# nimblephysics/nimblephysics

Hardware: AMD Instinct MI355X
Metric: worlds*timesteps/sec fwd+bwd (higher is better)
Workload: dtype f64; 1 GPU; Atlas 20-DOF (free root + 14 revolutes, arms welded) standing on the ground box, 8 frictional foot-corner contacts (24 LCP rows), pose q[0]=-pi/2 q[4]=-0.01 + N(0,0.02^2) joint noise; batch=4096 worlds/GPU; fwd+bwd through the C ABI, cold LCP start each step; ONE model handle in deferred-join mode (its slices run on the handle's own streams, the per-slice loss on them); n_dofs=20, contacts=8, lcp_rows=24, worlds_per_gpu=4096, saved_record_bytes_per_world_step=26720, rccl_world_size=0, devices_visible=1, device_of_rank0=0, gpu_max_hw_queues=4, collective=1 all-gather of the shared-control gradient per timed region

## Files before the change

nimblephysics_amd/csrc/coop_dantzig_dev.hpp:

```cpp
#pragma once
#include "coop_dev.hpp"

namespace NBL_NS {

template <int I> struct IntTag { static constexpr int value = I; };

DEV void coopPin24(double (&a)[MAXR]) {
#if defined(__HIP_DEVICE_COMPILE__)
  static_assert(MAXR % 8 == 0, "groups of eight");
#pragma unroll
  for (int g = 0; g < MAXR; g += 8)
    asm volatile("" : "+v"(a[g]), "+v"(a[g + 1]), "+v"(a[g + 2]), "+v"(a[g + 3]), "+v"(a[g + 4]), "+v"(a[g + 5]), "+v"(a[g + 6]), "+v"(a[g + 7]));
#endif
}

#if defined(NBL_CASCADE_TIMING) && defined(__HIPCC__)
__device__ unsigned long long g_dzStat[16];
__device__ unsigned long long g_dzStatSlow[16];
#ifndef NBL_DZ_SLOW
#define NBL_DZ_SLOW 300000
#endif
#endif
#if defined(NBL_CASCADE_TIMING) && defined(__HIP_DEVICE_COMPILE__)
#define DZ_T0() long long dzT = clock64(); long long dzAcc[12] = {0, 0, 0, 0, 0, 0, 0, 0, 0, 0, 0, 0}
#define DZ_ADD(k) do { const long long dzN = clock64(); dzAcc[k] += dzN - dzT; dzT = dzN; } while (0)
#define DZ_CNT(k) do { dzAcc[k] += 1; } while (0)
#define DZ_FLUSH() do { if (ln == 0) { long long dzTot = 0; for (int dzK = 0; dzK < 8; dzK++) dzTot += dzAcc[dzK];                      \
                                        for (int dzK = 0; dzK < 12; dzK++) atomicAdd(&g_dzStat[dzK], (unsigned long long)dzAcc[dzK]);           \
                                        if (dzTot > NBL_DZ_SLOW) for (int dzK = 0; dzK < 12; dzK++) atomicAdd(&g_dzStatSlow[dzK], (unsigned long long)dzAcc[dzK]); } } while (0)
#else
#define DZ_T0() do { } while (0)
#define DZ_ADD(k) do { } while (0)
#define DZ_CNT(k) do { } while (0)
#define DZ_FLUSH() do { } while (0)
#endif

struct PgsLds {
  double A[MAXR * CLD];
  double v[4][MAXR];
};

struct CascadeLds {
  double A[MAXR * CLD];
  double L[MAXR * CLD];
  double v[4][MAXR];
  double d[MAXR];
  int iv[2][MAXR];
};

struct CoopLcpRow {
  double x, b, lo, hi;
  int findex;
};

#if defined(__HIP_DEVICE_COMPILE__)
constexpr unsigned dzLanes(int from, int to) { return from >= to ? 0u : (unsigned)(((1ull << to) - 1ull) & ~((1ull << from) - 1ull)); }
template <unsigned SW>
DEV void dzSwitchStep(double& acc, double rhs, unsigned long long all) {
  asm volatile("s_mov_b64 exec, %[sw]\n\t"
               "v_add_f64 %[acc], %[rhs], -%[acc]\n\t"
               "s_mov_b64 exec, %[all]"
               : [acc] "+v"(acc)
               : [rhs] "v"(rhs), [sw] "n"(SW), [all] "s"(all));
}
template <unsigned YM, unsigned ZM>
DEV void dzSubstStep(double& acc, double l, double xk, unsigned long long all) {
  double t;
  if constexpr (YM != 0u && ZM != 0u) {
    asm volatile("v_mul_f64 %[t], %[l], %[xk]\n\t"
                 "s_mov_b64 exec, %[ym]\n\t"
                 "v_add_f64 %[acc], %[acc], -%[t]\n\t"
                 "s_mov_b64 exec, %[zm]\n\t"
                 "v_add_f64 %[acc], %[acc], %[t]\n\t"
                 "s_mov_b64 exec, %[all]"
                 : [acc] "+v"(acc), [t] "=&v"(t)
                 : [l] "v"(l), [xk] "s"(xk), [ym] "n"(YM), [zm] "n"(ZM), [all] "s"(all));
  } else if constexpr (YM != 0u) {
    asm volatile("v_mul_f64 %[t], %[l], %[xk]\n\t"
                 "s_mov_b64 exec, %[ym]\n\t"
                 "v_add_f64 %[acc], %[acc], -%[t]\n\t"
                 "s_mov_b64 exec, %[all]"
                 : [acc] "+v"(acc), [t] "=&v"(t)
                 : [l] "v"(l), [xk] "s"(xk), [ym] "n"(YM), [all] "s"(all));
  } else if constexpr (ZM != 0u) {
    asm volatile("v_mul_f64 %[t], %[l], %[xk]\n\t"
                 "s_mov_b64 exec, %[zm]\n\t"
                 "v_add_f64 %[acc], %[acc], %[t]\n\t"
                 "s_mov_b64 exec, %[all]"
                 : [acc] "+v"(acc), [t] "=&v"(t)
                 : [l] "v"(l), [xk] "s"(xk), [zm] "n"(ZM), [all] "s"(all));
  }
}
template <int K, class W>
DEV void dzL1BlockStep(const W& w, double& acc, double rhs, const double (&lrow)[MAXR], unsigned long long all) {
  if constexpr (K % 4 == 0) dzSwitchStep<dzLanes(K, K + 4)>(acc, rhs, all);
  const double xk = w.bcast(acc, K);
  dzSubstStep<dzLanes(K + 1, (K | 3) + 1), dzLanes((K | 3) + 1, 32)>(acc, lrow[K], xk, all);
}
template <int K, class W>
DEV void dzL1TailStep(const W& w, double& acc, double rhs, const double (&lrow)[MAXR], unsigned long long all) {
  dzSwitchStep<dzLanes(K, K + 1)>(acc, rhs, all);
  const double xk = w.bcast(acc, K);
  dzSubstStep<0u, dzLanes(K + 1, 32)>(acc, lrow[K], xk, all);
}
template <int J, class W>
DEV void dzL1Blocks(const W& w, double& acc, double rhs, const double (&lrow)[MAXR], int nC, int nb4, unsigned long long all) {
  if constexpr (4 * J < MAXR) {
    if (4 * J < nb4) {
      dzL1BlockStep<4 * J>(w, acc, rhs, lrow, all);
      dzL1BlockStep<4 * J + 1>(w, acc, rhs, lrow, all);
      dzL1BlockStep<4 * J + 2>(w, acc, rhs, lrow, all);
      dzL1BlockStep<4 * J + 3>(w, acc, rhs, lrow, all);
      dzL1Blocks<J + 1>(w, acc, rhs, lrow, nC, nb4, all);
    } else if (4 * J < nC) {
      dzL1TailStep<4 * J>(w, acc, rhs, lrow, all);
      if (4 * J + 1 < nC) {
        dzL1TailStep<4 * J + 1>(w, acc, rhs, lrow, all);
        if (4 * J + 2 < nC) dzL1TailStep<4 * J + 2>(w, acc, rhs, lrow, all);
      }
    }
  }
}
template <int RHO, int K, class W>
DEV void dzL1TBlockStep(const W& w, double& acc, double rhs, const double (&lcol)[MAXR], unsigned long long all) {
  constexpr int B0 = RHO + 4 * ((K - RHO) / 4);
  if constexpr (K == B0 + 3) dzSwitchStep<dzLanes(B0, B0 + 4)>(acc, rhs, all);
  const double xk = w.bcast(acc, K);
  dzSubstStep<dzLanes(B0, K), dzLanes(0, B0)>(acc, lcol[K], xk, all);
}
template <int K, class W>
DEV void dzL1TTailStep(const W& w, double& acc, double rhs, const double (&lcol)[MAXR], unsigned long long all) {
  dzSwitchStep<dzLanes(K, K + 1)>(acc, rhs, all);
  const double xk = w.bcast(acc, K);
  dzSubstStep<0u, dzLanes(0, K)>(acc, lcol[K], xk, all);
}
template <int RHO, int J, class W>
DEV void dzL1TBlocks(const W& w, double& acc, double rhs, const double (&lcol)[MAXR], int nC, unsigned long long all) {
  if constexpr (J >= 0) {
    if constexpr (RHO + 4 * J + 3 < MAXR) {
      if (RHO + 4 * J + 3 < nC) {
        dzL1TBlockStep<RHO, RHO + 4 * J + 3>(w, acc, rhs, lcol, all);
        dzL1TBlockStep<RHO, RHO + 4 * J + 2>(w, acc, rhs, lcol, all);
        dzL1TBlockStep<RHO, RHO + 4 * J + 1>(w, acc, rhs, lcol, all);
        dzL1TBlockStep<RHO, RHO + 4 * J>(w, acc, rhs, lcol, all);
      }
    }
    dzL1TBlocks<RHO, J - 1>(w, acc, rhs, lcol, nC, all);
  } else {
    if constexpr (RHO >= 3) dzL1TTailStep<2>(w, acc, rhs, lcol, all);
    if constexpr (RHO >= 2) dzL1TTailStep<1>(w, acc, rhs, lcol, all);
    if constexpr (RHO >= 1) dzL1TTailStep<0>(w, acc, rhs, lcol, all);
  }
}
#endif

template <class W>
DEV int coopDantzig(const W& w, CascadeLds& C, int n, CoopLcpRow& row) {
#if defined(__clang__)
#pragma clang fp contract(off)
#endif
  const int ln = w.lane();
  const bool on = ln < n;
  const int me = on ? ln : 0;
  DZ_T0();
  DZ_CNT(8);
  double x = 0.0, ww = 0.0, b = on ? row.b : 0.0, lo = on ? row.lo : 0.0, hi = on ? row.hi : 0.0, dx = 0.0, dw = 0.0;
  int st = 0, fidx = on ? row.findex : -1, p = me;
  int Cv = 0;
  double ell = 0.0, Dell = 0.0;
  int nC = 0, nN = 0;
  auto swapProblem = [&](int i1, int i2) {
    if (i1 == i2) return;
    if (on) { const double t = C.A[i1 * CLD + ln]; C.A[i1 * CLD + ln] = C.A[i2 * CLD + ln]; C.A[i2 * CLD + ln] = t; }
    w.sync();
    if (on) { const double t = C.A[ln * CLD + i1]; C.A[ln * CLD + i1] = C.A[ln * CLD + i2]; C.A[ln * CLD + i2] = t; }
    w.sync();
    const int src = ln == i1 ? i2 : (ln == i2 ? i1 : ln);
    x = w.shfl(x, src); b = w.shfl(b, src); ww = w.shfl(ww, src); lo = w.shfl(lo, src); hi = w.shfl(hi, src);
    p = w.shflI(p, src); st = w.shflI(st, src); fidx = w.shflI(fidx, src);
  };
  {
    const uint64_t fricBits = w.ballot(on && fidx >= 0);
    int atEnd = 0;
    for (int k = n - 1; k >= 0; k--) {
      if ((fricBits >> k) & 1ull) {
        const int i2 = n - 1 - atEnd;
        if (k != i2) {
          const int pk = w.bcastI(p, k), pi = w.bcastI(p, i2), fk = w.bcastI(fidx, k), f2 = w.bcastI(fidx, i2);
          const bool isK = ln == k, isI2 = ln == i2;
          p = isK ? pi : (isI2 ? pk : p);
          fidx = isK ? f2 : (isI2 ? fk : fidx);
        }
        atEnd++;
      }
    }
    double col[MAXR];
#pragma unroll
    for (int r = 0; r < MAXR; r++) {
      const int pr = w.bcastI(p, r < n ? r : 0);
      const int hiI = pr >= p ? pr : p, loI = pr >= p ? p : pr;
      const double av = C.A[hiI * CLD + loI];
      col[r] = (on && r < n) ? av : 0.0;
    }
    w.sync();
    if (ln < MAXR) {
#pragma unroll
      for (int r = 0; r < MAXR; r++) C.A[r * CLD + ln] = col[r];
    }
    b = w.shfl(b, p); lo = w.shfl(lo, p); hi = w.shfl(hi, p);
    w.sync();
  }
  auto seqRange = [&](double prod, int from, int to) -> double {
    double s = 0.0;
    int k = from;
#pragma unroll 1
    for (; k + 4 <= to; k += 4) {
      const double t0 = w.bcast(prod, k), t1 = w.bcast(prod, k + 1), t2 = w.bcast(prod, k + 2), t3 = w.bcast(prod, k + 3);
      s = s + t0; s = s + t1; s = s + t2; s = s + t3;
    }
#pragma unroll 1
    for (; k < to; k++) s = s + w.bcast(prod, k);
    return s;
  };
#ifdef NBL_SEQSUM_LDS
  auto seqSum2 = [&](double prod, int mid, int to, double& s1, double& s2) {
    w.sync();
    if (ln < MAXR) { C.v[2][ln] = ln < mid ? prod : 0.0; C.v[3][ln] = (ln >= mid && ln < to) ? prod : 0.0; }
    w.sync();
    s1 = 0.0; s2 = 0.0;
#pragma unroll
    for (int k4 = 0; k4 < MAXR; k4 += 4) {
      if (k4 < to) {
#pragma unroll
        for (int k = k4; k < k4 + 4; k++) { s1 = s1 + C.v[2][k]; s2 = s2 + C.v[3][k]; }
      }
    }
  };
#else
  auto seqSum2 = [&](double prod, int mid, int to, double& s1, double& s2) {
    s1 = seqRange(prod, 0, mid);
    s2 = seqRange(prod, mid, to);
  };
#endif
#ifdef NBL_SEQSUM_LDS
  auto seqSum = [&](double prod, int from, int to) -> double { double s1, s2; seqSum2(prod, to, to, s1, s2); return s1; };
#else
  auto seqSum = [&](double prod, int from, int to) -> double { return seqRange(prod, from, to); };
#endif
  auto solveL1 = [&](double rhs) -> double {
    const bool act = ln < nC;
    const int nb4 = nC & ~3;
    const int i0 = (ln < nb4) ? (ln & ~3) : ln;
    double lrow[MAXR];
#pragma unroll
    for (int k = 0; k < MAXR; k++) lrow[k] = C.L[me * CLD + k];
    coopPin24(lrow);
#if defined(__HIP_DEVICE_COMPILE__)
    if constexpr (MAXR <= 32) {
      double acc = 0.0;
      const unsigned long long all = __builtin_amdgcn_read_exec();
      dzL1Blocks<0>(w, acc, rhs, lrow, nC, nb4, all);
      return ln < nC ? acc : rhs;
    }
#endif
    double Z = 0.0, y = rhs;
#pragma unroll
    for (int k = 0; k < MAXR; k++) {
      if (k < nC) {
        if (k == i0) y = rhs - Z;
        const double xk = w.bcast(y, k);
        const double t = lrow[k] * xk;
        if (act && k < i0) Z = Z + t;
        if (k >= i0 && k < ln) y = y - t;
      }
    }
    return y;
  };
  auto solveL1T = [&](double rhs) -> double {
    const bool act = ln < nC;
    const int jr = nC - 1 - ln;
    const int nb4 = nC & ~3;
    const int i0 = (jr < nb4) ? (jr & ~3) : jr;
    double lcol[MAXR];
#pragma unroll
    for (int k = 0; k < MAXR; k++) lcol[k] = C.L[k * CLD + me];
    coopPin24(lcol);
#if defined(__HIP_DEVICE_COMPILE__)
    if constexpr (MAXR <= 32) {
      double acc = 0.0;
      const unsigned long long all = __builtin_amdgcn_read_exec();
      const int rho = nC & 3;
      constexpr int JTOP = MAXR / 4 - 1;
      if (rho == 0) dzL1TBlocks<0, JTOP>(w, acc, rhs, lcol, nC, all);
      else if (rho == 1) dzL1TBlocks<1, JTOP>(w, acc, rhs, lcol, nC, all);
      else if (rho == 2) dzL1TBlocks<2, JTOP>(w, acc, rhs, lcol, nC, all);
      else dzL1TBlocks<3, JTOP>(w, acc, rhs, lcol, nC, all);
      return ln < nC ? acc : rhs;
    }
#endif
    double Z = 0.0, y = rhs;
#pragma unroll
    for (int k = MAXR - 1; k >= 0; k--) {
      if (k < nC) {
        const int kr = nC - 1 - k;
        if (kr == i0) y = rhs - Z;
        const double xk = w.bcast(y, k);
        const double t = lcol[k] * xk;
        if (act && kr < i0) Z = Z + t;
        if (act && kr >= i0 && kr < jr) y = y - t;
      }
    }
    return y;
  };
  auto solveEll = [&](int i) {
    const double rhs = ln < nC ? C.A[i * CLD + Cv] : 0.0;
    Dell = solveL1(rhs);
    ell = ln < nC ? Dell * C.d[me] : 0.0;
  };
  auto solve1 = [&](int i, int dir) {
    if (nC == 0) return;
    solveEll(i);
    const double t = solveL1T(ell);
    w.sync();
    if (ln < nC) C.v[1][Cv] = dir > 0 ? -t : t;
    w.sync();
    dx = ln < nC ? C.v[1][me] : dx;
  };
  auto appendFactorRow = [&](int i) {
    const double aii = C.A[i * CLD + i];
    if (nC > 0) {
      if (ln < nC) C.L[nC * CLD + ln] = ell;
      const double dot = seqSum(ell * Dell, 0, nC);
      if (ln == 0) C.d[nC] = 1.0 / (aii - dot);
    } else if (ln == 0) C.d[0] = 1.0 / aii;
    w.sync();
  };
  auto ldltAddTL = [&](int r, int n2, double a) {
    const int nn = n2 - r;
    if (nn < 2) return;
    const bool act = ln >= r && ln < n2;
    const int pl = ln - r;
    const double SQ = 0.70710678118654752440;
    double W1 = (act && pl >= 1) ? a * SQ : 0.0, W2 = W1;
    const double a0 = w.bcast(a, r);
    const double W11 = (0.5 * a0 + 1.0) * SQ, W21 = (0.5 * a0 - 1.0) * SQ;
    double alpha1 = 1.0, alpha2 = 1.0;
    {
      double dee = C.d[r];
      double alphanew = alpha1 + (W11 * W11) * dee;
      dee /= alphanew;
      const double gamma1 = W11 * dee;
      dee *= alpha1;
      alpha1 = alphanew;
      alphanew = alpha2 - (W21 * W21) * dee;
      dee /= alphanew;
      alpha2 = alphanew;
      const double k1 = 1.0 - W21 * gamma1;
      const double k2 = W21 * gamma1 * W11 - W21;
      if (act && pl >= 1) {
        const double Wp = W1, el = C.L[me * CLD + r];
        W1 = Wp - W11 * el;
        W2 = k1 * Wp + k2 * el;
      }
    }
#pragma unroll 1
    for (int j = 1; j < nn; j++) {
      const double k1 = w.bcast(W1, r + j), k2 = w.bcast(W2, r + j);
      double dee = C.d[r + j];
      double alphanew = alpha1 + (k1 * k1) * dee;
      dee /= alphanew;
      const double gamma1 = k1 * dee;
      dee *= alpha1;
      alpha1 = alphanew;
      alphanew = alpha2 - (k2 * k2) * dee;
      dee /= alphanew;
      const double gamma2 = k2 * dee;
      dee *= alpha2;
      w.sync();
      if (ln == 0) C.d[r + j] = dee;
      alpha2 = alphanew;
      if (act && pl > j) {
        double el = C.L[me * CLD + r + j];
        double Wp = W1 - k1 * el;
        el += gamma1 * Wp;
        W1 = Wp;
        Wp = W2 - k2 * el;
        el -= gamma2 * Wp;
        W2 = Wp;
        C.L[me * CLD + r + j] = el;
      }
    }
    w.sync();
  };
  auto ldltRemove = [&](int n2, int r) {
    if (r == n2 - 1) return;
    const bool act = ln >= r && ln < n2;
    const int Cr = w.bcastI(Cv, r);
    const double ga = C.A[(act ? Cv : 0) * CLD + Cr];
    double a;
    if (r == 0) a = -ga;
    else {
      if (ln < r) C.v[2][ln] = C.L[r * CLD + ln] / C.d[ln];
      w.sync();
      double s = 0.0;
#pragma unroll 1
      for (int k = 0; k < r; k++) s = s + C.L[me * CLD + k] * C.v[2][k];
      a = s - ga;
    }
    if (ln == r) a += 1.0;
    ldltAddTL(r, n2, act ? a : 0.0);
    double lrow[MAXR];
    const int src = ln >= r ? ln + 1 : ln;
    const int srcc = src < MAXR ? src : MAXR - 1;
#pragma unroll
    for (int k = 0; k < MAXR; k++) lrow[k] = C.L[srcc * CLD + (k >= r ? (k + 1 < MAXR ? k + 1 : MAXR - 1) : k)];
    const double dsrc = C.d[srcc];
    w.sync();
    if (ln < n2 - 1) {
#pragma unroll
      for (int k = 0; k < MAXR; k++) C.L[ln * CLD + k] = lrow[k];
      C.d[ln] = dsrc;
    }
    w.sync();
  };
  auto removeFromC = [&](int i) {
    const int j = __builtin_ctzll(w.ballot(ln < nC && Cv == i));
    ldltRemove(nC, j);
    const int k = __builtin_ctzll(w.ballot(ln < nC && Cv == nC - 1));
    if (ln == k) Cv = i;
    const int cNext = w.shflI(Cv, ln + 1);
    if (ln >= j) Cv = cNext;
    swapProblem(i, nC - 1);
    nN++; nC--;
  };
  bool hitFirstFriction = false;
#ifdef NBL_DZ_COUNTS
  int dzIters = 0, dzRemovals = 0, dzTransfers = 0;
#endif
  DZ_ADD(0);
  for (int i = 0; i < n; ++i) {
    DZ_CNT(9);
    const int fi = w.bcastI(fidx, i);
    if (!hitFirstFriction && fi >= 0) {
      if (on) C.v[0][p] = x;
      w.sync();
      if (on && ln >= i) {
        const double wfk = C.v[0][fidx >= 0 ? fidx : 0];
        if (wfk == 0) { hi = 0; lo = 0; }
        else { hi = fabs(hi * wfk); lo = -hi; }
      }
      w.sync();
      hitFirstFriction = true;
    }
    {
      const double pr = on ? C.A[i * CLD + me] * x : 0.0;
      double sC, sN;
      seqSum2(pr, nC, nC + nN, sC, sN);
      const double s = sC + sN - w.bcast(b, i);
      if (ln == i) ww = s;
    }
    DZ_ADD(1);
    const double wi0 = w.bcast(ww, i), loi = w.bcast(lo, i), hii = w.bcast(hi, i);
    if (loi == 0 && wi0 >= 0) { if (ln == i) st = 0; nN++; }
    else if (hii == 0 && wi0 <= 0) { if (ln == i) st = 1; nN++; }
    else if (wi0 == 0) {
      if (nC > 0) solveEll(i);
      appendFactorRow(i); swapProblem(nC, i); if (ln == nC) Cv = nC; nC++;
    } else {
      for (;;) {
        const double wi = w.bcast(ww, i);
        const int dir = (wi <= 0) ? 1 : -1;
        const double dirf = dir;
        DZ_CNT(10);
#ifdef NBL_DZ_COUNTS
        dzIters++;
#endif
        solve1(i, dir);
        DZ_ADD(2);
        {
          double arow[MAXR];
#pragma unroll
          for (int j = 0; j < MAXR; j++) arow[j] = C.A[me * CLD + j];
          const double ai = C.A[me * CLD + i];
          coopPin24(arow);
          const double dxz = ln < nC ? dx : 0.0;
          double s = 0.0;
#pragma unroll
          for (int j4 = 0; j4 < MAXR; j4 += 4) {
            if (j4 < nC) {
              const double x0 = w.bcast(dxz, j4), x1 = w.bcast(dxz, j4 + 1), x2 = w.bcast(dxz, j4 + 2), x3 = w.bcast(dxz, j4 + 3);
              const double p0 = arow[j4] * x0, p1 = arow[j4 + 1] * x1, p2 = arow[j4 + 2] * x2, p3 = arow[j4 + 3] * x3;
              s = s + p0; s = s + p1; s = s + p2; s = s + p3;
            }
          }
          const bool inN = ln >= nC && ln < nC + nN;
          if (inN) dw = dir > 0 ? s + ai : s - ai;
          if (ln == i) dw = s + ai * dirf;
        }
        DZ_ADD(3);
        const bool inN = ln >= nC && ln < nC + nN, inC = ln < nC, isI = ln == i;
        const bool dn = dx < 0;
        const double num = (isI || inN) ? -ww : ((dn ? lo : hi) - x);
        const double den = (isI || inN) ? dw : dx;
        const double q = num / den;
        double s = INFINITY;
        int cmd = 0;
        if (isI) {
          s = q; cmd = 1;
          if (dir > 0) { if (hi < INFINITY) { const double s2 = (hi - x) * dirf; if (s2 < s) { s = s2; cmd = 3; } } }
          else { if (lo > -INFINITY) { const double s2 = (lo - x) * dirf; if (s2 < s) { s = s2; cmd = 2; } } }
        } else if (inN) {
          if (((st == 0) ? dw < 0 : dw > 0) && !(lo == 0 && hi == 0)) { s = q; cmd = 4; }
        } else if (inC) {
          if (dn && lo > -INFINITY) { s = q; cmd = 5; }
          if (dx > 0 && hi < INFINITY) { s = q; cmd = 6; }
        }
        const double sOwn = w.bcast(s, i);
        if (sOwn != sOwn) { row.x = 0.0; DZ_FLUSH(); return -1; }
        const double sMin = w.template minRows<MAXR>(cmd != 0 ? s : INFINITY);
        const uint64_t tie = w.ballot(cmd != 0 && s == sMin);
        if (tie == 0ull) { row.x = 0.0; DZ_FLUSH(); return -1; }
        int best;
        {
          const uint64_t mi = tie & (1ull << i);
          const uint64_t maskN = nN > 0 ? (((1ull << nN) - 1ull) << nC) : 0ull;
          const uint64_t maskC = nC > 0 ? ((1ull << nC) - 1ull) : 0ull;
          if (mi) best = i;
          else if (tie & maskN) best = __builtin_ctzll(tie & maskN);
          else best = __builtin_ctzll((tie & maskC) ? (tie & maskC) : tie);
        }
        const int cmdB = w.bcastI(cmd, best);
        if (sMin <= 0.0) { row.x = 0.0; DZ_FLUSH(); return 0; }
        const int si = best;
        DZ_ADD(4);
        if (ln < nC) x = x + sMin * dx;
        if (ln == i) x = x + sMin * dirf;
        if (ln >= nC && ln < nC + nN) ww = ww + sMin * dw;
        if (ln == i) ww = ww + sMin * dw;
        switch (cmdB) {
          case 1: if (ln == i) ww = 0; appendFactorRow(i); swapProblem(nC, i); if (ln == nC) Cv = nC; nC++; break;
          case 2: if (ln == i) { x = lo; st = 0; } nN++; break;
          case 3: if (ln == i) { x = hi; st = 1; } nN++; break;
          case 4:
            if (ln == si) ww = 0;
            if (nC > 0) solveEll(si);
            appendFactorRow(si); swapProblem(nC, si); if (ln == nC) Cv = nC; nN--; nC++; break;
          case 5: if (ln == si) { x = lo; st = 0; } removeFromC(si); break;
          case 6: if (ln == si) { x = hi; st = 1; } removeFromC(si); break;
        }
        if (cmdB >= 5) DZ_CNT(11);
#ifdef NBL_DZ_COUNTS
        if (cmdB >= 5) dzRemovals++;
        if (cmdB == 4) dzTransfers++;
#endif
        if (cmdB >= 5) DZ_ADD(7);
        else DZ_ADD(5);
        if (cmdB <= 3) break;
      }
    }
    DZ_ADD(6);
  }
  w.sync();
  if (on) C.v[0][p] = x;
  w.sync();
  row.x = on ? C.v[0][ln] : 0.0;
  w.sync();
  DZ_FLUSH();
#ifdef NBL_DZ_COUNTS
  row.x = ln == 0 ? (double)dzIters : (ln == 1 ? (double)dzRemovals : (ln == 2 ? (double)dzTransfers : 0.0));
#endif
  return 1;
}

template <class W, class LDS>
DEV void coopRemoveRow(const W& w, LDS& C, int n, int col, CoopLcpRow& row) {
  const int ln = w.lane();
  if (ln < n) for (int j = col; j + 1 < n; j++) C.A[ln * CLD + j] = C.A[ln * CLD + j + 1];
  w.sync();
  if (ln < n) for (int i = col; i + 1 < n; i++) C.A[i * CLD + ln] = C.A[(i + 1) * CLD + ln];
  w.sync();
  const double x1 = w.shfl(row.x, ln + 1), b1 = w.shfl(row.b, ln + 1), l1 = w.shfl(row.lo, ln + 1), h1 = w.shfl(row.hi, ln + 1);
  const int f1 = w.shflI(row.findex, ln + 1);
  if (ln >= col && ln + 1 < n) { row.x = x1; row.b = b1; row.lo = l1; row.hi = h1; row.findex = f1; }
}

template <class W, class LDS>
DEV int coopKeepRows(const W& w, LDS& C, int n, uint64_t keep, CoopLcpRow& row, int& mapTo) {
  const int ln = w.lane();
  const int nNew = __builtin_popcountll(keep);
  auto newIdx = [&](int p) -> int { return __builtin_popcountll(keep & ((1ull << p) - 1ull)); };
  const bool kept = ln < n && ((keep >> ln) & 1ull);
  w.sync();
  if (kept) C.v[0][newIdx(ln)] = (double)ln;
  w.sync();
  const int src = ln < nNew ? (int)C.v[0][ln] : 0;
  double col[MAXR];
  {
    uint64_t mm = keep;
#pragma unroll
    for (int j = 0; j < MAXR; j++) {
      if (j < nNew) {
        const int sj = __builtin_ctzll(mm);
        mm &= mm - 1ull;
        col[j] = C.A[src * CLD + sj];
      }
    }
  }
  w.sync();
  if (kept) { const int t = newIdx(ln); C.v[0][t] = row.x; C.v[1][t] = row.b; C.v[2][t] = row.lo; C.v[3][t] = row.hi; }
  const int fOld = w.shflI(row.findex, src);
  if (ln < nNew) {
#pragma unroll
    for (int j = 0; j < MAXR; j++) if (j < nNew) C.A[ln * CLD + j] = col[j];
  }
  w.sync();
  if (ln < nNew) {
    row.x = C.v[0][ln]; row.b = C.v[1][ln]; row.lo = C.v[2][ln]; row.hi = C.v[3][ln];
    row.findex = fOld >= 0 ? newIdx(fOld) : -1;
  }
  if (mapTo >= 0) mapTo = ((keep >> mapTo) & 1ull) ? newIdx(mapTo) : -1;
  w.sync();
  return nNew;
}

template <class W, class LDS>
DEV int coopLcpReduce(const W& w, LDS& C, int n, CoopLcpRow& row, int& mapTo) {
  const double TH = 1e-4;
  const int ln = w.lane();
  for (;;) {
    int ma = -1, mb = -1;
    for (int a = 0; a < n - 1; a++) {
      const double ba = w.bcast(row.b, a), ha = w.bcast(row.hi, a), la = w.bcast(row.lo, a);
      const int fa = w.bcastI(row.findex, a);
      const bool cand = ln > a && ln < n && fabs(ba - row.b) < TH && fa == row.findex && ha == row.hi && la == row.lo;
      if (w.ballot(cand) == 0ull) continue;
      double d2 = 0;
      const int bcol = ln < n ? ln : 0;
#pragma unroll
      for (int r = 0; r < MAXR; r++) {
        const double dr = C.A[r * CLD + a] - C.A[r * CLD + bcol];
        const double d = (r < n) ? dr : 0.0;
        d2 += d * d;
      }
      const uint64_t mm = w.ballot(cand && d2 < TH);
      if (mm) { ma = a; mb = __builtin_ctzll(mm); break; }
    }
    if (ma < 0) break;
    if (ln < n) C.A[ln * CLD + ma] *= 2.0;
    if (row.findex == mb) row.findex = ma;
    else if (row.findex > mb) row.findex -= 1;
    w.sync();
    coopRemoveRow(w, C, n, mb, row);
    n -= 1;
    if (mapTo == mb) mapTo = ma;
    else if (mapTo > mb) mapTo -= 1;
  }
  return n;
}

template <class W, class LDS>
DEV int coopLcpRemoveFriction(const W& w, LDS& C, int n, CoopLcpRow& row, int& mapTo) {
  const int ln = w.lane();
  return coopKeepRows(w, C, n, w.ballot(ln < n && row.findex == -1), row, mapTo);
}

#if defined(__HIP_DEVICE_COMPILE__)
#define NBL_PGS_OWN_NOFRIC                        \
        "s_mov_b64 exec, %[lane]\n\t"             \
        "v_add_f64 %[t0], %[x], %[r]\n\t"         \
        "v_max_f64 %[t0], %[t0], %[cL]\n\t"       \
        "v_min_f64 %[t0], %[t0], %[cH]\n\t"       \
        "v_add_f64 %[d], %[t0], -%[x]\n\t"        \
        "v_mov_b64 %[x], %[t0]\n\t"               \
        "s_mov_b64 exec, %[all]"
#define NBL_PGS_OWN_FRIC                          \
        "s_mov_b64 exec, %[lane]\n\t"             \
        "v_add_f64 %[t0], %[x], %[r]\n\t"         \
        "v_mul_f64 %[t1], %[cL], %[xf]\n\t"       \
        "v_max_f64 %[t0], %[t0], %[t1]\n\t"       \
        "v_mul_f64 %[t1], %[cH], %[xf]\n\t"       \
        "v_min_f64 %[t0], %[t0], %[t1]\n\t"       \
        "v_add_f64 %[d], %[t0], -%[x]\n\t"        \
        "v_mov_b64 %[x], %[t0]\n\t"               \
        "s_mov_b64 exec, %[all]"
template <int I, bool NOFRIC>
DEV void pgsOwnRow(double& x, double r, double xf, double cL, double cH, double& d, unsigned long long all) {
  double t0, t1;
  if constexpr (I < 32) {
    if constexpr (NOFRIC)
      asm volatile(NBL_PGS_OWN_NOFRIC : [x] "+v"(x), [d] "+v"(d), [t0] "=&v"(t0)
                   : [r] "v"(r), [cL] "v"(cL), [cH] "v"(cH), [lane] "n"(1u << (I & 31)), [all] "s"(all));
    else
      asm volatile(NBL_PGS_OWN_FRIC : [x] "+v"(x), [d] "+v"(d), [t0] "=&v"(t0), [t1] "=&v"(t1)
                   : [r] "v"(r), [xf] "v"(xf), [cL] "v"(cL), [cH] "v"(cH), [lane] "n"(1u << (I & 31)), [all] "s"(all));
  } else {
    const unsigned long long laneMask = 1ull << I;
    if constexpr (NOFRIC)
      asm volatile(NBL_PGS_OWN_NOFRIC : [x] "+v"(x), [d] "+v"(d), [t0] "=&v"(t0)
                   : [r] "v"(r), [cL] "v"(cL), [cH] "v"(cH), [lane] "s"(laneMask), [all] "s"(all));
    else
      asm volatile(NBL_PGS_OWN_FRIC : [x] "+v"(x), [d] "+v"(d), [t0] "=&v"(t0), [t1] "=&v"(t1)
                   : [r] "v"(r), [xf] "v"(xf), [cL] "v"(cL), [cH] "v"(cH), [lane] "s"(laneMask), [all] "s"(all));
  }
}
template <int I>
DEV void pgsFollowRow(double& xf, double& r, int fi, double ds, double narowI, unsigned long long all) {
  asm volatile("v_cmpx_eq_u32_e32 vcc, %[row], %[fi]\n\t"
               "s_nop 0\n\t"
               "v_add_f64 %[xf], %[xf], %[ds]\n\t"
               "s_mov_b64 exec, %[all]\n\t"
               "v_fmac_f64_e32 %[r], %[ds], %[na]"
               : [xf] "+v"(xf), [r] "+v"(r)
               : [fi] "v"(fi), [ds] "s"(ds), [na] "v"(narowI), [row] "n"(I), [all] "s"(all)
               : "vcc");
}
template <bool FIRST>
DEV bool pgsSweepBad(double x, double d, double thrFirst, double relTol, double epsDiv) {
  unsigned long long bad;
  if constexpr (FIRST) {
    asm volatile("v_cmp_gt_f64_e64 %[bad], |%[d]|, %[thr]" : [bad] "=s"(bad) : [d] "v"(d), [thr] "v"(thrFirst));
  } else {
    double t2;
    unsigned long long sc;
    asm volatile("v_mul_f64 %[t2], |%[x]|, %[rel]\n\t"
                 "v_cmp_gt_f64_e64 %[sc], |%[x]|, %[eps]\n\t"
                 "v_cmp_gt_f64_e64 %[bad], |%[d]|, %[t2]\n\t"
                 "s_and_b64 %[bad], %[bad], %[sc]"
                 : [bad] "=&s"(bad), [sc] "=&s"(sc), [t2] "=&v"(t2)
                 : [x] "v"(x), [d] "v"(d), [rel] "v"(relTol), [eps] "v"(epsDiv)
                 : "scc");
  }
  return bad != 0ull;
}
#else
template <int I, bool NOFRIC>
DEV void pgsOwnRow(double& x, double r, double xf, double cL, double cH, double& d, unsigned long long) {
  const double xi = NOFRIC ? fmin(fmax(x + r, cL), cH) : fmin(fmax(x + r, cL * xf), cH * xf);
  d = xi - x;
  x = xi;
}
template <int I>
DEV void pgsFollowRow(double& xf, double& r, int fi, double ds, double narowI, unsigned long long) {
  if (fi == I) xf += ds;
  r = fma(narowI, ds, r);
}
template <bool FIRST>
DEV bool pgsSweepBad(double x, double d, double thrFirst, double relTol, double epsDiv) {
  return FIRST ? fabs(d) > thrFirst : (fabs(x) > epsDiv && fabs(d) > relTol * fabs(x));
}
#endif

template <int I0, int I1, class F, class T>
DEV void pgsRowRange(F& rowStep, T tag) {
  if constexpr (I0 < I1) {
    rowStep(IntTag<I0>{}, tag);
    pgsRowRange<I0 + 1, I1>(rowStep, tag);
  }
}

template <bool NOFRIC = false, class W, class LDS>
DEV bool coopPgs(const W& w, LDS& C, int n, CoopLcpRow& row) {
  const int maxIteration = 30;
  const double dxTh = 1e-6, relTol = 1e-3, epsDiv = 1e-9;
  const int ln = w.lane();
  const bool on = ln < n;
  const int me = on ? ln : 0;
  double narow[MAXR];
#pragma unroll
  for (int j = 0; j < MAXR; j++) { const double av = C.A[me * CLD + j]; narow[j] = (on && j < n) ? av : 0.0; }
  const double aii = on ? C.A[me * CLD + me] : 1.0;
  const bool inOrder = on && !(aii < epsDiv);
  const double sc = inOrder ? 1.0 / aii : 1.0;
  const double nsc = -sc;
#pragma unroll
  for (int j = 0; j < MAXR; j++) narow[j] *= nsc;
  double x = on ? row.x : 0.0;
  double r0 = row.b * sc, r1 = 0.0;
#pragma unroll
  for (int j = 0; j < MAXR; j += 2) {
    r0 = fma(narow[j], j < n ? w.bcast(x, j) : 0.0, r0);
    r1 = fma(narow[j + 1], j + 1 < n ? w.bcast(x, j + 1) : 0.0, r1);
  }
  double r = r0 + r1;
  const int fi = on ? row.findex : -1;
  const bool fric = fi >= 0;
  const double cH = !inOrder ? 0.0 : row.hi, cL = !inOrder ? 0.0 : (fric ? -row.hi : row.lo);
  double xf = 1.0;
  if constexpr (!NOFRIC) {
    const double xNormal = w.shfl(x, fric ? fi : 0);
    xf = fric ? xNormal : 1.0;
  }
  const double thrFirst = inOrder ? dxTh : INFINITY;
  double d = 0.0;
#if defined(__HIP_DEVICE_COMPILE__)
  const unsigned long long all = __builtin_amdgcn_read_exec();
#else
  const unsigned long long all = 0ull;
#endif
  auto rowStep = [&](auto iTag, auto) {
    constexpr int i = decltype(iTag)::value;
#if defined(__HIP_DEVICE_COMPILE__)
    pgsOwnRow<i, NOFRIC>(x, r, xf, cL, cH, d, all);
#else
    if (ln == i) pgsOwnRow<i, NOFRIC>(x, r, xf, cL, cH, d, all);
#endif
    const double ds = w.bcast(d, i);
    if constexpr (NOFRIC) r = fma(narow[i], ds, r);
    else pgsFollowRow<i>(xf, r, fi, ds, narow[i], all);
  };
  auto sweep = [&](auto nTag) {
    constexpr int NR = decltype(nTag)::value;
    pgsRowRange<0, NR>(rowStep, IntTag<0>{});
  };
  auto noneBad = [&](auto firstTag) -> bool {
    constexpr bool first = decltype(firstTag)::value != 0;
#if defined(__HIP_DEVICE_COMPILE__)
    return !pgsSweepBad<first>(x, d, thrFirst, relTol, epsDiv);
#else
    return w.ballot(pgsSweepBad<first>(x, d, thrFirst, relTol, epsDiv)) == 0ull;
#endif
  };
  auto solve = [&](auto nTag) -> bool {
    sweep(nTag);
    if (noneBad(IntTag<1>{})) return true;
    bool done = false;
#pragma unroll 1
    for (int iter = 1; iter < maxIteration; ++iter) {
      sweep(nTag);
      if (noneBad(IntTag<0>{})) { done = true; break; }
    }
    return done;
  };
  bool done;
  if constexpr (NOFRIC) done = solve(IntTag<MAXR / 3>{});
  else done = n <= MAXR / 3 ? solve(IntTag<MAXR / 3>{}) : (n <= 2 * MAXR / 3 ? solve(IntTag<2 * MAXR / 3>{}) : solve(IntTag<MAXR>{}));
  row.x = x;
  return done;
}

struct CoopStageResult {
  double X;
  int flags;
};
constexpr int CS_SOLVED = 1;
constexpr int CS_VALID = 2;
constexpr int CS_NAN = 4;

template <class W, class LDS>
DEV void coopLoadProblem(const W& w, LDS& C, const CoopRow& R, double cfmDiag, double x0, CoopLcpRow& row, int& mapTo, int& nOut) {
  const int ln = w.lane();
  const int m = R.m;
  {
    double col[MAXR];
#pragma unroll
    for (int j = 0; j < MAXR; j++) col[j] = R.a(j);
    if (ln < m) {
#pragma unroll
      for (int j = 0; j < MAXR; j++) if (j < m) C.A[ln * CLD + j] = col[j] + (ln == j ? cfmDiag : 0.0);
    }
  }
  row.x = x0; row.b = R.Bv;
  row.lo = R.fric ? -R.mu : 0.0; row.hi = R.fric ? R.mu : INFINITY; row.findex = R.fric ? R.fp : -1;
  mapTo = ln < m ? ln : -1;
  w.sync();
  const RowMask dead = (RowMask)w.ballot(ln < m && (!R.on || (R.fric && R.mu == 0.0)));
  nOut = m;
  if (dead != 0) nOut = coopKeepRows(w, C, m, (uint64_t)w.ballot(ln < m) & ~(uint64_t)dead, row, mapTo);
}
template <class W, class LDS>
DEV double coopMapOut(const W& w, LDS& C, int m, int mapTo, double xred, int nred) {
  const int ln = w.lane();
  w.sync();
  if (ln < nred) C.v[3][ln] = xred;
  w.sync();
  return (ln < m && mapTo >= 0) ? C.v[3][mapTo] : 0.0;
}

template <class W>
DEV void coopCascadeStage1(const W& w, CascadeLds& C, const CoopRow& R, double X0, CoopStageResult& out) {
  CoopLcpRow row;
  int mapTo;
  int n0;
#if defined(NBL_CASCADE_TIMING) && defined(__HIP_DEVICE_COMPILE__)
  const int ln = w.lane();
  long long s1T = clock64();
#define S1_ADD(k) do { const long long n_ = clock64(); if (ln == 0) atomicAdd(&g_dzStat[k], (unsigned long long)(n_ - s1T)); s1T = n_; } while (0)
#else
#define S1_ADD(k) do { } while (0)
#endif
  coopLoadProblem(w, C, R, 0.0, X0, row, mapTo, n0);
  S1_ADD(12);
  const int nr = coopLcpReduce(w, C, n0, row, mapTo);
  S1_ADD(13);
  const int rc = coopDantzig(w, C, nr, row);
  S1_ADD(14);
  out.X = 0.0; out.flags = 0;
  if (rc == 1) {
    out.X = coopMapOut(w, C, R.m, mapTo, row.x, nr);
    out.flags = CS_SOLVED | (coopValid(w, C.v[0], R, out.X, false, 0.0) ? CS_VALID : 0);
  } else if (rc < 0) out.flags = CS_NAN;
  S1_ADD(15);
#undef S1_ADD
}
template <class W, class LDS>
DEV void coopCascadeStage2(const W& w, LDS& C, const CoopRow& R, double X0, double cfm, CoopStageResult& out) {
  CoopLcpRow row;
  int mapTo;
  int n0;
  coopLoadProblem(w, C, R, cfm, X0, row, mapTo, n0);
  const int nr = coopLcpReduce(w, C, n0, row, mapTo);
  out.X = 0.0; out.flags = 0;
  if (coopPgs(w, C, nr, row)) {
    out.X = coopMapOut(w, C, R.m, mapTo, row.x, nr);
    out.flags = CS_SOLVED | (coopValid(w, C.v[0], R, out.X, false, cfm) ? CS_VALID : 0);
  }
}
template <class W, class LDS>
DEV void coopCascadeStage3(const W& w, LDS& C, const CoopRow& R, double X0, double cfm, CoopStageResult& out) {
  CoopLcpRow row;
  int mapTo;
  int n0;
  coopLoadProblem(w, C, R, cfm, X0, row, mapTo, n0);
  const int nr = coopLcpRemoveFriction(w, C, n0, row, mapTo);
  row.x = 0.0;
  const bool ok3 = coopPgs<true>(w, C, nr, row);
  out.X = coopMapOut(w, C, R.m, mapTo, row.x, nr);
  out.flags = ok3 ? CS_SOLVED : 0;
}

struct CoopCascadeOut {
  double X;
  CoopClasses K;
  double cfm;
  uint32_t st;
  bool pinvValid;
};

template <class W>
DEV void coopCascadeChoose(const W& w, int m, double X0, double fallbackCfm, const CoopStageResult& r1, const CoopStageResult& r2,
                           const CoopStageResult& r3, double& X, double& cfm, bool& ignoreFriction, uint32_t& st) {
  const int ln = w.lane();
  auto hasNan = [&](double x) -> bool { return w.ballot(ln < m && x != x) != 0ull; };
  bool success = false;
  st = 0; ignoreFriction = false; cfm = 0.0; X = X0;
  if (r1.flags & CS_SOLVED) {
    X = r1.X;
    success = (r1.flags & CS_VALID) != 0;
    if (success) st |= 0x4u;
  }
  if ((r1.flags & CS_NAN) || hasNan(X)) { success = false; X = 0.0; st |= 0x40u; }
  if (!success) {
    cfm = fallbackCfm;
    if (r2.flags & CS_SOLVED) {
      X = r2.X;
      success = (r2.flags & CS_VALID) != 0;
      if (success) st |= 0x8u;
    }
  }
  if (!success) {
    ignoreFriction = true;
    X = r3.X;
    st |= 0x10u;
    if (!(r3.flags & CS_SOLVED)) st |= 0x20u;
  }
  if (hasNan(X)) { X = 0.0; st |= 0x40u; }
}

template <class W>
DEV void coopCascadeSelect(const W& w, CoopLds& S, const CoopRow& R, double X0, double fallbackCfm, const CoopStageResult& r1,
                           const CoopStageResult& r2, const CoopStageResult& r3, CoopCascadeOut& out) {
  double X, cfm;
  bool ignoreFriction;
  uint32_t st;
  coopCascadeChoose(w, R.m, X0, fallbackCfm, r1, r2, r3, X, cfm, ignoreFriction, st);
  bool pinvValid = false;
  const bool std = coopStandardizeLoop(w, S, R, X, cfm, ignoreFriction, 0u, pinvValid, out.K);
  if (std) st |= 0x100u;
  out.X = X; out.cfm = cfm; out.st = st; out.pinvValid = pinvValid;
}

}
```

Before: 7.312 million worlds*timesteps/s.

## Keep each lane's LDLT factor row and diagonal resident in registers during Dantzig

Each lane now keeps its own row of the L factor and its diagonal entry in registers, updated on append, remove and rank-2 update. This replaces the per-solve reload of L rows and the d reads from LDS. ldltRemove computes its dot product with cross-lane broadcasts instead of an LDS scratch vector, which drops one barrier, and the rank-2 update loop drops its per-iteration sync. The cost is higher register pressure from a persistent array of MAXR doubles, which could reduce occupancy or cause spills, plus extra code to keep the register and LDS copies consistent.

```diff
diff --git a/nimblephysics_amd/csrc/coop_dantzig_dev.hpp b/nimblephysics_amd/csrc/coop_dantzig_dev.hpp
--- a/nimblephysics_amd/csrc/coop_dantzig_dev.hpp
+++ b/nimblephysics_amd/csrc/coop_dantzig_dev.hpp
@@ -169,6 +169,11 @@
   int Cv = 0;
   double ell = 0.0, Dell = 0.0;
   int nC = 0, nN = 0;
+  constexpr bool kRegRow = MAXR <= 32;
+  double Lr[MAXR];
+#pragma unroll
+  for (int k = 0; k < MAXR; k++) Lr[k] = 0.0;
+  double dL = 0.0;
   auto swapProblem = [&](int i1, int i2) {
     if (i1 == i2) return;
     if (on) { const double t = C.A[i1 * CLD + ln]; C.A[i1 * CLD + ln] = C.A[i2 * CLD + ln]; C.A[i2 * CLD + ln] = t; }
@@ -251,10 +256,12 @@
     const bool act = ln < nC;
     const int nb4 = nC & ~3;
     const int i0 = (ln < nb4) ? (ln & ~3) : ln;
-    double lrow[MAXR];
-#pragma unroll
-    for (int k = 0; k < MAXR; k++) lrow[k] = C.L[me * CLD + k];
-    coopPin24(lrow);
+    double (&lrow)[MAXR] = Lr;
+    if constexpr (!kRegRow) {
+#pragma unroll
+      for (int k = 0; k < MAXR; k++) lrow[k] = C.L[me * CLD + k];
+      coopPin24(lrow);
+    }
 #if defined(__HIP_DEVICE_COMPILE__)
     if constexpr (MAXR <= 32) {
       double acc = 0.0;
@@ -315,7 +322,8 @@
   auto solveEll = [&](int i) {
     const double rhs = ln < nC ? C.A[i * CLD + Cv] : 0.0;
     Dell = solveL1(rhs);
-    ell = ln < nC ? Dell * C.d[me] : 0.0;
+    if constexpr (kRegRow) ell = ln < nC ? Dell * dL : 0.0;
+    else ell = ln < nC ? Dell * C.d[me] : 0.0;
   };
   auto solve1 = [&](int i, int dir) {
     if (nC == 0) return;
@@ -328,12 +336,26 @@
   };
   auto appendFactorRow = [&](int i) {
     const double aii = C.A[i * CLD + i];
+    double dNew;
     if (nC > 0) {
       if (ln < nC) C.L[nC * CLD + ln] = ell;
       const double dot = seqSum(ell * Dell, 0, nC);
-      if (ln == 0) C.d[nC] = 1.0 / (aii - dot);
-    } else if (ln == 0) C.d[0] = 1.0 / aii;
-    w.sync();
+      dNew = 1.0 / (aii - dot);
+    } else dNew = 1.0 / aii;
+    if (ln == 0) C.d[nC] = dNew;
+    w.sync();
+    if constexpr (kRegRow) {
+      if (ln == nC) dL = dNew;
+#pragma unroll
+      for (int k8 = 0; k8 < MAXR; k8 += 8) {
+        if (k8 < nC) {
+          if (ln == nC) {
+#pragma unroll
+            for (int k = k8; k < k8 + 8; k++) Lr[k] = C.L[nC * CLD + k];
+          }
+        }
+      }
+    }
   };
   auto ldltAddTL = [&](int r, int n2, double a) {
     const int nn = n2 - r;
@@ -346,7 +368,9 @@
     const double W11 = (0.5 * a0 + 1.0) * SQ, W21 = (0.5 * a0 - 1.0) * SQ;
     double alpha1 = 1.0, alpha2 = 1.0;
     {
-      double dee = C.d[r];
+      double dee;
+      if constexpr (kRegRow) dee = w.bcast(dL, r);
+      else dee = C.d[r];
       double alphanew = alpha1 + (W11 * W11) * dee;
       dee /= alphanew;
       const double gamma1 = W11 * dee;
@@ -362,6 +386,38 @@
         W1 = Wp - W11 * el;
         W2 = k1 * Wp + k2 * el;
       }
+    }
+    if constexpr (kRegRow) {
+#pragma unroll 1
+      for (int j = 1; j < nn; j++) {
+        const double elIn = C.L[me * CLD + r + j];
+        const double k1 = w.bcast(W1, r + j), k2 = w.bcast(W2, r + j);
+        double dee = w.bcast(dL, r + j);
+        double alphanew = alpha1 + (k1 * k1) * dee;
+        dee /= alphanew;
+        const double gamma1 = k1 * dee;
+        dee *= alpha1;
+        alpha1 = alphanew;
+        alphanew = alpha2 - (k2 * k2) * dee;
+        dee /= alphanew;
+        const double gamma2 = k2 * dee;
+        dee *= alpha2;
+        if (ln == 0) C.d[r + j] = dee;
+        if (ln == r + j) dL = dee;
+        alpha2 = alphanew;
+        if (act && pl > j) {
+          double el = elIn;
+          double Wp = W1 - k1 * el;
+          el += gamma1 * Wp;
+          W1 = Wp;
+          Wp = W2 - k2 * el;
+          el -= gamma2 * Wp;
+          W2 = Wp;
+          C.L[me * CLD + r + j] = el;
+        }
+      }
+      w.sync();
+      return;
     }
 #pragma unroll 1
     for (int j = 1; j < nn; j++) {
@@ -399,7 +455,26 @@
     const double ga = C.A[(act ? Cv : 0) * CLD + Cr];
     double a;
     if (r == 0) a = -ga;
-    else {
+    else if constexpr (kRegRow) {
+      const double lri = C.L[r * CLD + (ln < r ? ln : 0)];
+      const double ti = ln < r ? lri / dL : 0.0;
+      double s = 0.0;
+#pragma unroll
+      for (int k4 = 0; k4 < MAXR; k4 += 4) {
+        if (k4 + 4 <= r) {
+          const double t0 = w.bcast(ti, k4), t1 = w.bcast(ti, k4 + 1), t2 = w.bcast(ti, k4 + 2), t3 = w.bcast(ti, k4 + 3);
+          const double p0 = Lr[k4] * t0, p1 = Lr[k4 + 1] * t1, p2 = Lr[k4 + 2] * t2, p3 = Lr[k4 + 3] * t3;
+          s = s + p0; s = s + p1; s = s + p2; s = s + p3;
+        } else if (k4 < r) {
+          s = s + Lr[k4] * w.bcast(ti, k4);
+          if (k4 + 1 < r) {
+            s = s + Lr[k4 + 1] * w.bcast(ti, k4 + 1);
+            if (k4 + 2 < r) s = s + Lr[k4 + 2] * w.bcast(ti, k4 + 2);
+          }
+        }
+      }
+      a = s - ga;
+    } else {
       if (ln < r) C.v[2][ln] = C.L[r * CLD + ln] / C.d[ln];
       w.sync();
       double s = 0.0;
@@ -409,9 +484,32 @@
     }
     if (ln == r) a += 1.0;
     ldltAddTL(r, n2, act ? a : 0.0);
-    double lrow[MAXR];
     const int src = ln >= r ? ln + 1 : ln;
     const int srcc = src < MAXR ? src : MAXR - 1;
+    if constexpr (kRegRow) {
+#pragma unroll
+      for (int k8 = 0; k8 < MAXR; k8 += 8) {
+        if (k8 < n2) {
+#pragma unroll
+          for (int k = k8; k < k8 + 8; k++) Lr[k] = C.L[srcc * CLD + (k >= r ? (k + 1 < MAXR ? k + 1 : MAXR - 1) : k)];
+        }
+      }
+      dL = C.d[srcc];
+      w.sync();
+#pragma unroll
+      for (int k8 = 0; k8 < MAXR; k8 += 8) {
+        if (k8 < n2) {
+          if (ln < n2 - 1) {
+#pragma unroll
+            for (int k = k8; k < k8 + 8; k++) C.L[ln * CLD + k] = Lr[k];
+          }
+        }
+      }
+      if (ln < n2 - 1) C.d[ln] = dL;
+      w.sync();
+      return;
+    }
+    double lrow[MAXR];
 #pragma unroll
     for (int k = 0; k < MAXR; k++) lrow[k] = C.L[srcc * CLD + (k >= r ? (k + 1 < MAXR ? k + 1 : MAXR - 1) : k)];
     const double dsrc = C.d[srcc];
```

Result: slower. 7.103 million worlds*timesteps/s (-2.9%).
